# eradiate/eradiate-kernel

Measured on AMD Instinct MI355X. Metric: Msamples/s volpath 512x512x1024spp plane-parallel atmosphere, higher is better.
Workload: dtype f32; 1 GPU; C3 volpath heterogeneous 128^3 grid + HG g=0.8, 512x512x1024spp; integrator=volpath, sampler=independent seed 0, block_size=32, rfilter=box

## Files before the change

eradiate-kernel_amd/csrc/volpath_flat.h:

```cpp
#pragma once
#include "integrator_dev.h"

namespace mtsamd {
inline namespace MTS_VARIANT_NS {

#if MTS_SPEC_N == 3
#define MTS_CX
#define MTS_CXI(id)
#define MTS_SPEC_DW 3
#else
#define MTS_CX , cx
#define MTS_CXI(id) , cx, (id)
#define MTS_SPEC_DW 4
#endif

#if MTS_SPEC_N == 3
#define MTS_FILM_STRIDE(sc) ((size_t) 5)
#else
#define MTS_FILM_STRIDE(sc) ((size_t) (sc).film_channels)
#endif
#ifndef MTS_CHAIN
#define MTS_CHAIN 1
#endif
#ifndef MTS_REPEAT_MIN_W
// ... 140 lines not shown
        if (COUNT) cnt.n_lookup++;
        if (COUNT) MTS_SEG(cnt, 2);
    }
    mi.combined = combined;
    mi.inv_combined = inv_mext;
    mi.info = (m_homogeneous ? MI_HOMOGENEOUS : 0u) | (m_spectral ? MI_SPECTRAL : 0u) |
              (m.sample_emitters ? MI_SAMPLE_EMITTERS : 0u) | (m_grey ? MI_GREY : 0u) | ((uint32_t) m.phase << MI_PHASE_SHIFT);
    return mi;
}

DEV Spec transmittance_exp_g(float t, Spec combined, bool grey) {
    if (grey) return spec_s(pm_exp(-t * combined.x));
    return transmittance_exp(t, combined);
}

#if MTS_SPEC_N == 3
template <bool OWN_ATOMIC>
DEV void splat_sample_t(const DScene &sc, const DBlock &blk, uint32_t lx, uint32_t ly, F2 position_sample, F3 L, bool valid,
                        MTS_GLOBAL_AS float *film, float *own) {
    const DSensor &se = sc.sensor;
    float v[5];
    v[0] = pm_fma(0.180423f, L.z, pm_fma(0.357580f, L.y, 0.412453f * L.x));
    v[1] = pm_fma(0.072169f, L.z, pm_fma(0.715160f, L.y, 0.212671f * L.x));
    v[2] = pm_fma(0.950227f, L.z, pm_fma(0.119193f, L.y, 0.019334f * L.x));
    if (sc.integrator.monochrome)
        v[0] = v[1] = v[2] = L.x;
    v[3] = valid ? 1.f : 0.f;
    v[4] = 1.f;
    bool ok = true;
    for (int k = 0; k < 5; ++k) ok = ok && v[k] >= -1e-5f && pm_isfinite(v[k]);
    if (!ok) return;
    const DRFilter &rf = se.rfilter;
    const int border = rf.border_size;
    const int sx = blk.sx + 2 * border, sy = blk.sy + 2 * border;
    float posx = position_sample.x - ((float) (blk.ox - border) + .5f), posy = position_sample.y - ((float) (blk.oy - border) + .5f);
    if (rf.radius > 0.5f + MTS_RAY_EPSILON) {
        int lox = max((int) pm_ceil(posx - rf.radius), 0), loy = max((int) pm_ceil(posy - rf.radius), 0);
        int hix = min((int) pm_floor(posx + rf.radius), sx - 1), hiy = min((int) pm_floor(posy + rf.radius), sy - 1);
        uint32_t n = (uint32_t) pm_ceil((rf.radius - 2.f * MTS_RAY_EPSILON) * 2.f);
        float basex = (float) lox - posx, basey = (float) loy - posy;
        for (uint32_t yr = 0; yr < n; ++yr) {
            int y = loy + (int) yr;
            if (y > hiy) break;
            float wy = as_global(rf.values)[min((int) pm_abs((basey + (float) yr) * rf.scale_factor), 31)];
            int fy = blk.oy - border + y - se.crop_y;
            for (uint32_t xr = 0; xr < n; ++xr) {
                int x = lox + (int) xr;
                if (x > hix) break;
                float wx = as_global(rf.values)[min((int) pm_abs((basex + (float) xr) * rf.scale_factor), 31)];
                float weight = wy * wx;
                int fx = blk.ox - border + x - se.crop_x;
                if (fx >= 0 && fy >= 0 && fx < se.crop_w && fy < se.crop_h) {
                    float *dst = (float *) (film + 5 * ((size_t) fy * se.crop_w + fx));
                    for (int k = 0; k < 5; ++k) atomicAdd(dst + k, v[k] * weight);
                }
            }
        }
    } else {
        int lox = (int) pm_ceil(posx - .5f), loy = (int) pm_ceil(posy - .5f);
        if (lox == (int) lx && loy == (int) ly) {
            if (OWN_ATOMIC) { for (int k = 0; k < 5; ++k) atomicAdd(own + k, v[k]); }
            else { for (int k = 0; k < 5; ++k) own[k] += v[k]; }
        } else if (lox >= 0 && loy >= 0 && lox < sx && loy < sy) {
            float *dst = (float *) (film + 5 * ((size_t) (blk.oy + loy - se.crop_y) * se.crop_w + (blk.ox + lox - se.crop_x)));
            for (int k = 0; k < 5; ++k) atomicAdd(dst + k, v[k]);
        }
    }
}

#endif

struct PathState {
    Pcg32 rng;
    DRay ray;
    Hit si;
    int medium;
    Spec thr, res; float eta; uint32_t depth, channel;
    Spec trans; float wa, wb;
#if MTS_SPEC_N != 3
    Spec wl;
#endif
    uint32_t st, mode, flags;
};
enum { C_POS = 0,
       C_RAYW = 2,
       C_SO = 3, C_SD = 6,
       C_SHIT = 9,
       C_SMED = 17,
       C_CW = 18,
       C_EMIT = C_CW + MTS_SPEC_DW,
       C_ACC = C_EMIT + MTS_SPEC_DW,
       C_SAMPLE = C_ACC + 5,
       C_COUNT = C_SAMPLE + 1 };
static_assert(C_COUNT <= 32, "the cold record is one 128-byte line");
#define MTS_COLD_RECORD 32
template <class Ptr , bool AOS = false>
struct ColdStoreT {
    Ptr base; uint32_t stride;
    DEV auto &f(int k) const { return AOS ? base[k] : base[(size_t) k * stride]; }
    DEV void put3(int k, F3 v) const { f(k) = v.x; f(k + 1) = v.y; f(k + 2) = v.z; }
    DEV F3 get3(int k) const { return f3(f(k), f(k + 1), f(k + 2)); }
#if MTS_SPEC_N == 3
    DEV void put_spec(int k, Spec v) const { put3(k, v); }
    DEV Spec get_spec(int k) const { return get3(k); }
#else
    DEV void put_spec(int k, Spec v) const { f(k) = v.x; f(k + 1) = v.y; f(k + 2) = v.z; f(k + 3) = v.w; }
    DEV Spec get_spec(int k) const { return spec4(f(k), f(k + 1), f(k + 2), f(k + 3)); }
#endif
    DEV void put_hit(const Hit &h) const {
        f(C_SHIT) = h.t; put3(C_SHIT + 1, h.p); f(C_SHIT + 4) = h.uv.x; f(C_SHIT + 5) = h.uv.y;
        f(C_SHIT + 6) = __int_as_float(h.shape); f(C_SHIT + 7) = __int_as_float(h.prim);
    }
    DEV Hit get_hit() const {
        Hit h; h.t = f(C_SHIT); h.p = get3(C_SHIT + 1); h.uv.x = f(C_SHIT + 4); h.uv.y = f(C_SHIT + 5);
        h.shape = __float_as_int(f(C_SHIT + 6)); h.prim = __float_as_int(f(C_SHIT + 7)); return h;
    }
};
typedef ColdStoreT<float *> ColdStore;
typedef ColdStoreT<MTS_GLOBAL_AS float *, true> ColdStoreHbm;
template <class Cold>
struct PathEnvT {
    DBlock blk; uint32_t lx, ly, sample_count; MTS_GLOBAL_AS float *film; Cold cold;
    MTS_GLOBAL_AS float *park;
    uint32_t index;
};
enum { B_INT = 0, B_MED , B_SCATTER, B_WSURF, B_SURF, B_PHASE, B_NEW,
       B_MEDW , B_DONE, B_COUNT };

template <bool COUNT>
struct VolpathMachine {
    const DScene &sc;
    Counters &cnt;
    DEV VolpathMachine(const DScene &sc_, Counters &cnt_) : sc(sc_), cnt(cnt_) {}
#if MTS_SPEC_N == 3
    DEV SpecCtx ctx(const PathState &) const { return SpecCtx(); }
#else
    DEV SpecCtx ctx(const PathState &p) const { SpecCtx cx = make_ctx(sc); cx.wl = p.wl; return cx; }
#endif

    DEV void queue_intersection(PathState &p) const {
        float bmint, bmaxt;
        bbox_ray_intersect(sc.bbox, p.ray, bmint, bmaxt);
        p.si.t = pm_inf();
        if (pm_max(p.ray.mint, bmint) <= bmaxt) p.flags |= FL_NEEDS_INT; else p.flags &= ~FL_NEEDS_INT;
    }
    template <class E> DEV void begin_sample(PathState &p, const E &e) const {
        const DSensor &se = sc.sensor;
        const float px = (float) (e.lx + (uint32_t) e.blk.ox), py = (float) (e.ly + (uint32_t) e.blk.oy);
        if (se.wavefront) seed_wavefront_sample(p.rng, se, e.blk, e.lx, e.ly, __float_as_uint(e.cold.f(C_SAMPLE)));
        F2 u = p.rng.next_2d();
        F2 position_sample; position_sample.x = px + u.x; position_sample.y = py + u.y;
        F2 aperture_sample; aperture_sample.x = .5f; aperture_sample.y = .5f;
        if (se.needs_aperture_sample) aperture_sample = p.rng.next_2d();
        if (se.shutter_open_time > 0.f) (void) p.rng.next_1d();
#if MTS_SPEC_N == 3
        (void) p.rng.next_1d();
#else
        {
            const float wavelength_sample = p.rng.next_1d();
            float wav_weight; Spec srf_weight;
            p.wl = sc.srf >= 0 ? sample_wavelengths_srf(sc, wavelength_sample, srf_weight) : sample_wavelengths(wavelength_sample, wav_weight);
        }
#endif
        F2 adjusted;
        adjusted.x = (position_sample.x - (float) se.crop_x) / (float) se.crop_w;
        adjusted.y = (position_sample.y - (float) se.crop_y) / (float) se.crop_h;
        F3 rw;
        p.ray = sensor_sample_ray(sc, adjusted, aperture_sample, rw);
        e.cold.f(C_POS) = position_sample.x; e.cold.f(C_POS + 1) = position_sample.y; e.cold.f(C_RAYW) = rw.x;
        p.medium = se.medium;
        p.thr = spec_s(1.f); p.res = spec_s(0.f); p.eta = 1.f; p.depth = 0;
#if MTS_SPEC_N == 3
        p.channel = sc.integrator.monochrome ? 0u : (uint32_t) pm_min(p.rng.next_1d() * 3.f, 2.f);
#else
        p.channel = 0u;
#endif
        p.si.p = f3s(0.f); p.si.uv.x = p.si.uv.y = 0.f; p.si.prim = 0;
        const bool hide_emitters = sc.integrator.hide_emitters != 0;
        p.flags = FL_ALIVE | ((!hide_emitters && sc.environment >= 0) ? FL_VALID_RAY : 0u) | (!hide_emitters ? FL_SPEC_CHAIN : 0u);
        p.trans = spec_s(1.f); p.wa = p.wb = 0.f;
        queue_intersection(p);
        p.mode = M_MAIN; p.st = S_TOP;
    }
    template <class E> DEV void end_nee(PathState &p, const E &e) const {
        Spec emitted = p.trans * e.cold.get_spec(C_EMIT);
        p.res = p.res + e.cold.get_spec(C_CW) * emitted;
        p.mode = M_MAIN; p.medium = __float_as_int(e.cold.f(C_SMED));
        F3 d = e.cold.get3(C_SD);
        p.ray.d = d; p.ray.d_rcp = vrcp(d);
        if (p.flags & FL_FROM_MEDIUM) { p.ray.o = e.cold.get3(C_SO); p.st = S_PHASE; }
        else { p.si = e.cold.get_hit(); p.st = S_BSDF; }
    }
    template <class E> DEV void end_direct(PathState &p, const E &e, Spec emitter_val, float emitter_pdf) const {
        Spec emitted = p.trans * emitter_val;
        if (emitter_pdf != 0.f) p.res = p.res + mis_weight(p.wb, emitter_pdf) * p.thr * emitted;
        p.ray = spawn_ray(e.cold.get3(C_SO), e.cold.get3(C_SD));
        p.si = e.cold.get_hit(); p.medium = __float_as_int(e.cold.f(C_SMED));
        p.flags = (p.flags & ~FL_NEEDS_INT) | FL_ALIVE;
        p.mode = M_MAIN; p.st = S_TOP;
    }

    template <bool DEFER = false, class E> DEV void top(PathState &p, const E &e) const {
        if (p.st != S_TOP) return;
        const uint32_t max_depth = (uint32_t) sc.integrator.max_depth, rr_depth = (uint32_t) sc.integrator.rr_depth;
        if (p.mode == M_MAIN) {
            bool active = (p.flags & FL_ALIVE) && any_nonzero(p.thr);
            float q = pm_min(hmax(p.thr) * (p.eta * p.eta), .95f);
            bool perform_rr = p.depth > rr_depth;
            active = active && (p.rng.next_1d() < q || !perform_rr);
            if (perform_rr) p.thr = p.thr * pm_rcp(q);
            if (!active || p.depth >= max_depth) p.st = S_NEW;
            else { if (COUNT) cnt.n_iter++; p.st = p.medium >= 0 ? S_MED : S_SURF; }
        } else if (p.mode == M_NEE) {
            float remaining_dist = p.wb * (1.f - MTS_SHADOW_EPSILON) - p.wa;
            p.ray.maxt = remaining_dist;
            if (!(remaining_dist > 0.f)) { if (DEFER) p.st = S_ENDNEE; else end_nee(p, e); }
            else { if (COUNT) cnt.n_nee_step++; p.st = p.medium >= 0 ? S_MED : S_SURF; }
        } else {
            if (COUNT) cnt.n_nee_step++;
            p.st = p.medium >= 0 ? S_MED : S_SURF;
        }
    }
    DEV static bool wants_int(const PathState &p) { return (p.st == S_MED || p.st == S_SURF || p.st == S_DIRB) && (p.flags & FL_NEEDS_INT); }
    DEV static int classify(const PathState &p) {
        if (p.st == S_DONE) return B_DONE;
        if (wants_int(p)) return B_INT;
        if (p.st == S_MED) return p.mode == M_MAIN ? B_MED : B_MEDW;
        if (p.st == S_SCATTER) return B_SCATTER;
        if (p.st == S_SURF) return p.mode == M_MAIN ? B_SURF : B_WSURF;
        if (p.st == S_BSDF) return B_SURF;
        if (p.st == S_PHASE) return B_PHASE;
        return B_NEW;
    }

    template <class E> DEV void blk_new(PathState &p, const E &e) const {
        if (p.st != S_NEW) return;
        const DSensor &se = sc.sensor;
        F2 position_sample; position_sample.x = e.cold.f(C_POS); position_sample.y = e.cold.f(C_POS + 1);
        float acc[5];
        for (int k = 0; k < 5; ++k) acc[k] = e.cold.f(C_ACC + k);
#if MTS_SPEC_N == 3
        splat_sample_t<false>(sc, e.blk, e.lx, e.ly, position_sample, f3s(e.cold.f(C_RAYW)) * p.res, (p.flags & FL_VALID_RAY) != 0, e.film, acc);
#else
        {
            float wav_weight; (void) sample_wavelengths(0.f, wav_weight);
            const Spec ww = sc.srf >= 0 ? srf_weights_of(sc, p.wl) : spec_s(wav_weight);
            const Spec L = (ww * e.cold.f(C_RAYW)) * p.res;
            float xyz[3];
            spectrum_to_xyz(sc.cie, L, p.wl, xyz);
            const float v[5] = { xyz[0], xyz[1], xyz[2], (p.flags & FL_VALID_RAY) != 0 ? 1.f : 0.f, 1.f };
            if (sc.bin_count == 0) splat_values_t<false>(sc, e.blk, e.lx, e.ly, position_sample, v, e.film, acc);
            else splat_values_bins(sc, e.blk, e.lx, e.ly, position_sample, v, p.res, p.wl, e.film, acc);
        }
#endif
        const uint32_t sample_idx = __float_as_uint(e.cold.f(C_SAMPLE)) + 1u;
        if (sample_idx == e.sample_count) {
            float *own = (float *) (e.film + MTS_FILM_STRIDE(sc) * ((size_t) (e.blk.oy + (int) e.ly - se.crop_y) * se.crop_w + (e.blk.ox + (int) e.lx - se.crop_x)));
            for (int k = 0; k < 5; ++k) atomicAdd(own + k, acc[k]);
            p.st = S_DONE;
        } else {
            for (int k = 0; k < 5; ++k) e.cold.f(C_ACC + k) = acc[k];
            e.cold.f(C_SAMPLE) = __uint_as_float(sample_idx);
            begin_sample(p, e);
        }
    }
    template <class E> DEV void blk_int(PathState &p, const E &e) const {
        if (!wants_int(p)) return;
        p.si = ray_intersect(sc, p.ray);
        p.flags &= ~FL_NEEDS_INT;
        start_direct(p, e);
    }
    template <class E> DEV void start_direct(PathState &p, const E &e) const {
        if (p.st != S_DIRB || (p.flags & FL_NEEDS_INT)) return;
// ... 23 lines not shown
        const Spec sigma_n = homogeneous ? spec_s(0.f) : mi.combined - mi.sigma_t;
        const uint32_t channel = p.channel;
        const bool is_main = MODEK == 0 ? true : (MODEK == 1 ? false : p.mode == M_MAIN), is_nee = MODEK == 0 ? false : p.mode == M_NEE;
        const float remaining_dist = is_nee ? p.ray.maxt : pm_inf();
        Spec weight = is_main ? p.thr : p.trans;
        if (spectral) {
            float t = pm_min(mi.t, p.si.t);
            if (is_nee) t = pm_min(remaining_dist, t);
            t = t - mi.mint;
            const bool surface_first = p.si.t < mi.t || mi.t > remaining_dist;
            if (grey || !homogeneous) {
                float tr = pm_exp(-t * mi.combined.x);
                float tr_pdf = surface_first ? tr : tr * mi.combined.x;
                weight = weight * (tr_pdf > 0.f ? tr * pm_rcp(tr_pdf) : 0.f);
            } else {
                Spec tr = transmittance_exp(t, mi.combined);
                Spec free_flight_pdf = surface_first ? tr : tr * mi.combined;
                float tr_pdf = pick(free_flight_pdf, channel);
                weight = weight * (tr_pdf > 0.f ? tr / tr_pdf : spec_s(0.f));
            }
        }
        float u2 = 0.f;
        if (is_main) u2 = p.rng.next_1d();
        if (is_nee) {
            if (mi.t > remaining_dist && mi.t != pm_inf()) p.wa = p.wb;
            if (mi.t > remaining_dist) mi.t = pm_inf();
        }
        const bool valid = mi.t != pm_inf();
        if (!valid) {
            if (is_main) p.thr = weight; else p.trans = weight;
            p.st = S_SURF;
            return;
        }
        const bool real_scatter = is_main && !(u2 >= (grey ? div_by_invariant(mi.sigma_t.x, mi.combined.x, mi.inv_combined)
                                                                : div_by_invariant(pick(mi.sigma_t, channel), pick(mi.combined, channel), mi.inv_combined)));
        if (!real_scatter) {
            if (grey) {
                if (is_main) { if (spectral) weight = weight * ((sigma_n.x * mi.combined.x) * pm_rcp(sigma_n.x)); }
                else { if (spectral) weight = weight * sigma_n.x; else weight = weight * div_by_invariant(sigma_n.x, mi.combined.x, mi.inv_combined); }
            } else {
                if (is_main) { if (spectral) weight = weight * (sigma_n * pick(mi.combined, channel) / pick(sigma_n, channel)); }
                else { if (spectral) weight = weight * sigma_n; else weight = weight * div_by_invariant(sigma_n, mi.combined, mi.inv_combined); }
            }
            if (is_nee) p.wa += mi.t;
            p.ray.o = mi.p; p.ray.mint = 0.f; p.si.t = p.si.t - mi.t;
            p.st = S_TOP;
            if (is_main) p.thr = weight;
            else {
                p.trans = weight;
                if (!any_nonzero(weight)) {
                    if (DEFER) p.st = is_nee ? S_ENDNEE : S_ENDDIR0;
                    else if (is_nee) end_nee(p, e); else end_direct(p, e, spec_s(0.f), 0.f);
                }
            }
            return;
        }
        p.depth += 1;
        if (!(p.depth < max_depth)) { p.thr = weight; p.flags &= ~FL_ALIVE; p.st = S_TOP; return; }
        if (grey) {
            if (spectral) weight = weight * ((mi.sigma_s.x * mi.combined.x) * pm_rcp(mi.sigma_t.x));
            else weight = weight * (mi.sigma_s.x / mi.sigma_t.x);
        } else {
            if (spectral) weight = weight * (mi.sigma_s * pick(mi.combined, channel) / pick(mi.sigma_t, channel));
            else weight = weight * (mi.sigma_s / mi.sigma_t);
        }
        p.thr = weight;
        const bool sample_emitters = (mi.info & MI_SAMPLE_EMITTERS) != 0;
        p.flags |= FL_VALID_RAY;
        p.flags = sample_emitters ? (p.flags & ~FL_SPEC_CHAIN) : (p.flags | FL_SPEC_CHAIN);
        p.ray.o = mi.p;
        p.st = sample_emitters ? S_SCATTER : S_PHASE;
    }
    template <class E> DEV void blk_scatter(PathState &p, const E &e) const {
        if (p.st != S_SCATTER) return;
        p.st = S_PHASE;
        Spec emitter_val;
        const SpecCtx cx = ctx(p); (void) cx;
        DirSample ds = sample_emitter_direction(sc, p.ray.o, p.rng.next_2d(), false, emitter_val MTS_CX);
        if (ds.pdf == 0.f) return;
        float phase_val = 0.f;
        WATERFALL_BEGIN(p.medium, mu)
            phase_val = phase_eval<true>(sc, cload(sc.media + mu).phase, -p.ray.d, p.ray.o, ds.d MTS_CX);
        WATERFALL_END
        e.cold.put_spec(C_CW, p.thr * phase_val); e.cold.put_spec(C_EMIT, emitter_val);
        e.cold.put3(C_SO, p.ray.o); e.cold.put3(C_SD, p.ray.d); e.cold.f(C_SMED) = __int_as_float(p.medium);
        p.trans = spec_s(1.f); p.wa = 0.f; p.wb = ds.dist;
        p.ray = spawn_ray(p.ray.o, ds.d); p.ray.mint = 0.f;
        queue_intersection(p);
        p.flags |= FL_FROM_MEDIUM;
        p.mode = M_NEE; p.st = S_TOP;
    }
    template <class E> DEV void blk_wsurf(PathState &p, const E &e) const {
        if (p.st != S_SURF || p.mode == M_MAIN || (p.flags & FL_NEEDS_INT)) return;
        const bool hit = hit_valid(p.si);
        const bool is_nee = p.mode == M_NEE;
        if (is_nee) p.wa += p.si.t;
        int emitter = is_nee ? -1 : sc.environment;
        Surf sf; sf.wi = -p.ray.d; sf.sh.n = f3s(0.f); sf.n = f3s(0.f);
        Spec nt = spec_s(0.f); int is_tr = 0, ext = -1, inte = -1;
        if (hit) {
            WATERFALL_BEGIN(p.si.shape, su)
                const DShape s = cload(sc.shapes + su);
                if (!is_nee) emitter = s.emitter;
                nt = s.bsdf_type == MTS_BSDF_NULL ? spec_s(1.f) : spec_s(0.f);
                is_tr = s.is_medium_transition; ext = s.exterior; inte = s.interior;
                if (emitter >= 0) complete_surface(sc, s, p.si, p.ray.d, sf);
                else if (is_tr) sf.n = hit_geo_normal(sc, s, p.si);
            WATERFALL_END
        }
        if (emitter >= 0) {
            const F3 ref_p = e.cold.get3(C_SO);
            DirSample ds;
            ds.p = p.si.p; ds.n = sf.sh.n; ds.d = p.si.p - ref_p; ds.dist = norm(ds.d); ds.d = ds.d / ds.dist;
            if (!hit) ds.d = -sf.wi;
            ds.emitter = emitter; ds.pdf = 0.f; ds.delta = false;
            const SpecCtx cx = ctx(p); (void) cx;
            end_direct(p, e, emitter_eval(sc, emitter, sf.wi.z MTS_CX), pdf_emitter_direction(sc, ref_p, ds));
            return;
        }
        if (hit) {
            p.trans = p.trans * nt;
            p.ray = spawn_ray(p.si.p, p.ray.d);
            queue_intersection(p);
            if (is_tr) p.medium = dot(p.ray.d, sf.n) > 0 ? ext : inte;
        }
        if (hit && any_nonzero(p.trans)) p.st = S_TOP;
        else if (is_nee) end_nee(p, e);
        else end_direct(p, e, spec_s(0.f), 0.f);
    }
    template <class E> DEV void blk_surf(PathState &p, const E &e) const {
        if (p.st != S_SURF || p.mode != M_MAIN || (p.flags & FL_NEEDS_INT)) return;
        const uint32_t max_depth = (uint32_t) sc.integrator.max_depth;
        const bool hit = hit_valid(p.si);
        Surf sf; sf.wi = -p.ray.d; sf.n = f3s(0.f); sf.sh.s = sf.sh.t = sf.sh.n = f3s(0.f);
        int emitter = sc.environment, bsdf_id = 0;
        if (hit) {
            WATERFALL_BEGIN(p.si.shape, su)
                const DShape s = cload(sc.shapes + su);
                emitter = s.emitter; bsdf_id = s.bsdf;
                if (s.emitter >= 0 || (s.bsdf_flags & F_Smooth) != 0) complete_surface(sc, s, p.si, p.ray.d, sf);
            WATERFALL_END
        }
        const SpecCtx cx = ctx(p); (void) cx;
        if ((p.flags & FL_SPEC_CHAIN) && emitter >= 0) p.res = p.res + p.thr * emitter_eval(sc, emitter, sf.wi.z MTS_CX);
        if (!hit) { p.flags &= ~FL_ALIVE; p.st = S_TOP; return; }
        p.st = S_BSDF;
        bool active_e = false;
        WATERFALL_BEGIN(bsdf_id, bu)
            active_e = (cload(sc.bsdfs + bu).flags & F_Smooth) != 0 && (p.depth + 1 < max_depth);
        WATERFALL_END
        if (!active_e) return;
        Spec emitter_val;
        DirSample ds = sample_emitter_direction(sc, p.si.p, p.rng.next_2d(), false, emitter_val MTS_CX);
        if (ds.pdf == 0.f) return;
        F3 wo = to_local(sf.sh, ds.d);
        Spec bsdf_val; float bpdf;
        WATERFALL_BEGIN(bsdf_id, bu)
            const DBsdf bsdf = cload(sc.bsdfs + bu);
            bsdf_val = bsdf_eval(bsdf, sf.wi, wo MTS_CXI(bu));
            bpdf = bsdf_pdf(bsdf, sf.wi, wo MTS_CXI(bu));
        WATERFALL_END
        e.cold.put_spec(C_CW, p.thr * bsdf_val * mis_weight(ds.pdf, ds.delta ? 0.f : bpdf)); e.cold.put_spec(C_EMIT, emitter_val);
        e.cold.put_hit(p.si); e.cold.put3(C_SD, p.ray.d); e.cold.f(C_SMED) = __int_as_float(p.medium);
        p.trans = spec_s(1.f); p.wa = 0.f; p.wb = ds.dist;
        p.ray = spawn_ray(p.si.p, ds.d);
        queue_intersection(p);
        p.flags &= ~FL_FROM_MEDIUM;
        p.mode = M_NEE; p.st = S_TOP;
    }
    template <class E> DEV void blk_bsdf(PathState &p, const E &e) const {
        if (p.st != S_BSDF) return;
        const uint32_t max_depth = (uint32_t) sc.integrator.max_depth;
        Surf sf; int bsdf_id = 0, is_tr = 0, ext = -1, inte = -1;
        WATERFALL_BEGIN(p.si.shape, su)
            const DShape s = cload(sc.shapes + su);
            complete_surface(sc, s, p.si, p.ray.d, sf);
            bsdf_id = s.bsdf; is_tr = s.is_medium_transition; ext = s.exterior; inte = s.interior;
        WATERFALL_END
        const float s1 = p.rng.next_1d(); const F2 s2 = p.rng.next_2d();
        BSDFSample bs; Spec bsdf_val;
        const SpecCtx cx = ctx(p); (void) cx;
        WATERFALL_BEGIN(bsdf_id, bu)
            const DBsdf bsdf = cload(sc.bsdfs + bu);
            bsdf_val = bsdf_sample(bsdf, sf.wi, s1, s2, bs MTS_CXI(bu));
        WATERFALL_END
        p.thr = p.thr * bsdf_val;
        p.eta *= bs.eta;
        p.ray = spawn_ray(p.si.p, to_world(sf.sh, bs.wo));
        p.flags |= FL_ALIVE;
        const bool non_null_bsdf = !(bs.sampled_type & F_Null);
        if (non_null_bsdf) { p.depth += 1; p.flags |= FL_VALID_RAY; }
        if (non_null_bsdf && (bs.sampled_type & F_Delta)) p.flags |= FL_SPEC_CHAIN;
        if (bs.sampled_type & F_Smooth) p.flags &= ~FL_SPEC_CHAIN;
        const bool add_emitter = !(bs.sampled_type & F_Delta) && any_nonzero(p.thr) && (p.depth < max_depth);
        const int new_medium = is_tr ? (dot(p.ray.d, sf.n) > 0 ? ext : inte) : p.medium;
        queue_intersection(p);
        if (add_emitter) { e.cold.f(C_SMED) = __int_as_float(new_medium); p.wb = bs.pdf; p.st = S_DIRB; start_direct(p, e); }
        else { p.medium = new_medium; p.st = S_TOP; }
    }
    template <class E> DEV void blk_phase(PathState &p, const E &e) const {
        if (p.st != S_PHASE) return;
        const float s1 = p.rng.next_1d(); const F2 s2 = p.rng.next_2d();
        F3 wo;
        const SpecCtx cx = ctx(p); (void) cx;
        WATERFALL_BEGIN(p.medium, mu)
            wo = phase_sample<true>(sc, cload(sc.media + mu).phase, make_frame(p.ray.d), p.ray.o, s1, s2 MTS_CX);
        WATERFALL_END
        p.ray = spawn_ray(p.ray.o, wo); p.ray.mint = 0.0f;
        queue_intersection(p);
        p.flags |= FL_ALIVE;
        p.st = S_TOP;
    }

    template <class E> DEV void finish(PathState &p, const E &e) const {
        if (p.st == S_ENDNEE) end_nee(p, e);
        else if (p.st == S_ENDDIR0) end_direct(p, e, spec_s(0.f), 0.f);
    }
    template <bool DEFER = false, bool SPLIT = false, class E> DEV void run(PathState &p, const E &e, int sel) const {
        switch (sel) {
            case B_NEW: blk_new(p, e); break;
            case B_INT: blk_int(p, e); break;
            case B_MED: if (SPLIT) blk_med<DEFER, 0>(p, e); else blk_med<DEFER, -1>(p, e); break;
            case B_MEDW: if (SPLIT) blk_med<DEFER, 1>(p, e); else blk_med<DEFER, -1>(p, e); break;
            case B_SCATTER: blk_scatter(p, e); break;
            case B_WSURF: blk_wsurf(p, e); break;
            case B_SURF: blk_surf(p, e); blk_bsdf(p, e); break;
            case B_PHASE: blk_phase(p, e); break;
            default: break;
        }
    }
};

#if MTS_SPEC_N == 3
template <bool COUNT>
DEV void volpath_pixel_flat(const DScene &sc, Pcg32 &rng, const DBlock &blk, uint32_t lx, uint32_t ly, uint32_t sample_count,
                            float *__restrict__ film, ColdStore cold, Counters &cnt, const uint32_t *stop_flag) {
    VolpathMachine<COUNT> vm(sc, cnt);
    PathEnvT<ColdStore> e; e.blk = blk; e.lx = lx; e.ly = ly; e.sample_count = sample_count; e.film = as_global(film); e.cold = cold;
    PathState p; p.rng = rng;
    for (int k = 0; k < 5; ++k) e.cold.f(C_ACC + k) = 0.f;
    e.cold.f(C_SAMPLE) = __uint_as_float(0u);
    vm.begin_sample(p, e);
#if defined(MTSAMD_BLOCKSTATS)
    long long bs_t0 = clock64(); int bs_prev_sel = 20;
    unsigned long long bs_loc[45] = {};
// ... 516 lines not shown
```

eradiate-kernel_amd/csrc/volpathmis_flat.h:

```cpp
#pragma once
#include "volpath_flat.h"

namespace mtsamd {
inline namespace MTS_VARIANT_NS {

#if MTS_SPEC_N == 3
DEV int c_pdfv(bool) { return 30; }
#else
DEV int c_pdfv(bool from_medium) { return from_medium ? C_SHIT : C_SO; }
#endif

template <bool SPEC>
struct MisPathState {
    Pcg32 rng;
    DRay ray; Hit si; int medium;
    MisWeights<SPEC> pf, pn;
    MisWeights<SPEC> wn, wu;
    Spec res; F3 lsp;
#if MTS_SPEC_N != 3
    Spec wl;
#endif
    float eta, wa, wb;
    uint32_t depth, channel, st, mode, flags;
};

template <bool COUNT, bool SPEC>
struct VolpathMisMachine {
    typedef MisPathState<SPEC> P;
    typedef MisWeights<SPEC> W;
    const DScene &sc;
    Counters &cnt;
    DEV VolpathMisMachine(const DScene &sc_, Counters &cnt_) : sc(sc_), cnt(cnt_) {}
#if MTS_SPEC_N == 3
    DEV SpecCtx ctx(const P &) const { return SpecCtx(); }
#else
    DEV SpecCtx ctx(const P &p) const { SpecCtx cx = make_ctx(sc); cx.wl = p.wl; return cx; }
#endif

    DEV void queue_intersection(P &p) const {
        float bmint, bmaxt;
        bbox_ray_intersect(sc.bbox, p.ray, bmint, bmaxt);
        p.si.t = pm_inf();
        if (pm_max(p.ray.mint, bmint) <= bmaxt) p.flags |= FL_NEEDS_INT; else p.flags &= ~FL_NEEDS_INT;
    }
    template <class E> DEV static void park_put(const E &e, const W &a, const W &b) {
        constexpr int NR = SPEC ? MTS_SPEC_N : 1;
        for (int i = 0; i < NR; ++i) {
            MTS_GLOBAL_AS float *pa = e.park + MTS_SPEC_N * i, *pb = e.park + MTS_SPEC_N * (NR + i);
            pa[0] = a.r[i].x; pa[1] = a.r[i].y; pa[2] = a.r[i].z; pb[0] = b.r[i].x; pb[1] = b.r[i].y; pb[2] = b.r[i].z;
#if MTS_SPEC_N != 3
            pa[3] = a.r[i].w; pb[3] = b.r[i].w;
#endif
        }
    }
    template <class E> DEV static void park_get(const E &e, W &a, W &b) {
        constexpr int NR = SPEC ? MTS_SPEC_N : 1;
        for (int i = 0; i < NR; ++i) {
            const MTS_GLOBAL_AS float *pa = e.park + MTS_SPEC_N * i, *pb = e.park + MTS_SPEC_N * (NR + i);
            a.r[i].x = pa[0]; a.r[i].y = pa[1]; a.r[i].z = pa[2]; b.r[i].x = pb[0]; b.r[i].y = pb[1]; b.r[i].z = pb[2];
#if MTS_SPEC_N != 3
            a.r[i].w = pa[3]; b.r[i].w = pb[3];
#endif
        }
    }
    DEV bool walk_goes_on(const P &p) const {
        if (SPEC) return any_nonzero(mis_weight_w(p.wu));
        return any_nonzero(p.wu.r[0]) || any_nonzero(p.wn.r[0]);
    }
    template <class E> DEV void begin_sample(P &p, const E &e) const {
        const DSensor &se = sc.sensor;
        const float px = (float) (e.lx + (uint32_t) e.blk.ox), py = (float) (e.ly + (uint32_t) e.blk.oy);
        if (se.wavefront) seed_wavefront_sample(p.rng, se, e.blk, e.lx, e.ly, __float_as_uint(e.cold.f(C_SAMPLE)));
        F2 u = p.rng.next_2d();
        F2 position_sample; position_sample.x = px + u.x; position_sample.y = py + u.y;
        F2 aperture_sample; aperture_sample.x = .5f; aperture_sample.y = .5f;
        if (se.needs_aperture_sample) aperture_sample = p.rng.next_2d();
        if (se.shutter_open_time > 0.f) (void) p.rng.next_1d();
#if MTS_SPEC_N == 3
        (void) p.rng.next_1d();
#else
        {
            const float wavelength_sample = p.rng.next_1d();
            float wav_weight; Spec srf_weight;
            p.wl = sc.srf >= 0 ? sample_wavelengths_srf(sc, wavelength_sample, srf_weight) : sample_wavelengths(wavelength_sample, wav_weight);
        }
#endif
        F2 adjusted;
        adjusted.x = (position_sample.x - (float) se.crop_x) / (float) se.crop_w;
        adjusted.y = (position_sample.y - (float) se.crop_y) / (float) se.crop_h;
        F3 rw;
        p.ray = sensor_sample_ray(sc, adjusted, aperture_sample, rw);
        e.cold.f(C_POS) = position_sample.x; e.cold.f(C_POS + 1) = position_sample.y; e.cold.f(C_RAYW) = rw.x;
        p.medium = se.medium;
        p.res = spec_s(0.f); p.lsp = f3s(0.f); p.eta = 1.f; p.depth = 0;
        p.pf = mw_full<SPEC>(1.f); p.pn = mw_full<SPEC>(1.f); p.wn = mw_full<SPEC>(1.f); p.wu = mw_full<SPEC>(1.f);
#if MTS_SPEC_N == 3
        p.channel = sc.integrator.monochrome ? 0u : (uint32_t) pm_min(p.rng.next_1d() * 3.f, 2.f);
#else
        p.channel = 0u;
#endif
        p.si.p = f3s(0.f); p.si.uv.x = p.si.uv.y = 0.f; p.si.prim = 0; p.si.shape = -1;
        const bool hide_emitters = sc.integrator.hide_emitters != 0;
        p.flags = FL_ALIVE | ((!hide_emitters && sc.environment >= 0) ? FL_VALID_RAY : 0u) | (!hide_emitters ? FL_SPEC_CHAIN : 0u);
        p.wa = p.wb = 0.f;
        queue_intersection(p);
        p.mode = M_MAIN; p.st = S_TOP;
    }
    template <class E> DEV void end_nee(P &p, const E &e) const {
        const Spec fval = e.cold.get_spec(C_CW), emitted = e.cold.get_spec(C_EMIT);
        const float pdfv = e.cold.f(c_pdfv((p.flags & FL_FROM_MEDIUM) != 0));
        update_weights(p.wn, 1.0f, fval, p.channel, true);
        update_weights(p.wu, pdfv, fval, p.channel, true);
        p.res = p.res + mis_weight_w(p.wn, p.wu) * emitted;
        park_get(e, p.pf, p.pn);
        p.mode = M_MAIN; p.medium = __float_as_int(e.cold.f(C_SMED));
        F3 d = e.cold.get3(C_SD);
        p.ray.d = d; p.ray.d_rcp = vrcp(d);
        if (p.flags & FL_FROM_MEDIUM) { p.ray.o = e.cold.get3(C_SO); p.st = S_PHASE; }
        else { p.si = e.cold.get_hit(); p.st = S_BSDF; }
    }
    template <bool DEFER, class E> DEV void nee_done(P &p, const E &e) const { if (DEFER) p.st = S_ENDNEE; else end_nee(p, e); }
    template <class E> DEV void finish(P &p, const E &e) const { if (p.st == S_ENDNEE) end_nee(p, e); }
    template <bool DEFER = false, class E> DEV void top(P &p, const E &e) const {
        if (p.st != S_TOP) return;
        const uint32_t max_depth = (uint32_t) sc.integrator.max_depth, rr_depth = (uint32_t) sc.integrator.rr_depth;
        if (p.mode == M_MAIN) {
            bool active = (p.flags & FL_ALIVE) != 0;
            Spec mis_throughput = mis_weight_w(p.pf);
            float q = pm_min(hmax(mis_throughput) * (p.eta * p.eta), .95f);
            bool perform_rr = active && (p.depth > rr_depth);
            active = active && !(p.rng.next_1d() >= q && perform_rr);
            update_weights(p.pf, q, 1.0f, p.channel, perform_rr);
            active = active && !(p.depth >= max_depth);
            active = active && any_nonzero(mis_weight_w(p.pf));
            if (!active) p.st = S_NEW;
            else { if (COUNT) cnt.n_iter++; p.st = p.medium >= 0 ? S_MED : S_SURF; }
        } else {
            float remaining_dist = p.wb * (1.f - MTS_SHADOW_EPSILON) - p.wa;
            p.ray.maxt = remaining_dist;
            if (!(remaining_dist > 0.f)) nee_done<DEFER>(p, e);
            else { if (COUNT) cnt.n_nee_step++; p.st = p.medium >= 0 ? S_MED : S_SURF; }
        }
    }
    DEV static bool wants_int(const P &p) { return (p.st == S_MED || p.st == S_SURF) && (p.flags & FL_NEEDS_INT); }
    DEV static int classify(const P &p) {
        if (p.st == S_DONE) return B_DONE;
        if (wants_int(p)) return B_INT;
        if (p.st == S_MED) return p.mode == M_MAIN ? B_MED : B_MEDW;
        if (p.st == S_SCATTER) return B_SCATTER;
        if (p.st == S_SURF) return p.mode == M_MAIN ? B_SURF : B_WSURF;
        if (p.st == S_BSDF) return B_SURF;
        if (p.st == S_PHASE) return B_PHASE;
        return B_NEW;
    }

    template <class E> DEV void blk_new(P &p, const E &e) const {
        if (p.st != S_NEW) return;
        const DSensor &se = sc.sensor;
        F2 position_sample; position_sample.x = e.cold.f(C_POS); position_sample.y = e.cold.f(C_POS + 1);
        float acc[5];
        for (int k = 0; k < 5; ++k) acc[k] = e.cold.f(C_ACC + k);
#if MTS_SPEC_N == 3
        splat_sample_t<false>(sc, e.blk, e.lx, e.ly, position_sample, f3s(e.cold.f(C_RAYW)) * p.res, (p.flags & FL_VALID_RAY) != 0, e.film, acc);
#else
        {
            float wav_weight; (void) sample_wavelengths(0.f, wav_weight);
            const Spec ww = sc.srf >= 0 ? srf_weights_of(sc, p.wl) : spec_s(wav_weight);
            const Spec L = (ww * e.cold.f(C_RAYW)) * p.res;
            float xyz[3];
            spectrum_to_xyz(sc.cie, L, p.wl, xyz);
            const float v[5] = { xyz[0], xyz[1], xyz[2], (p.flags & FL_VALID_RAY) != 0 ? 1.f : 0.f, 1.f };
            if (sc.bin_count == 0) splat_values_t<false>(sc, e.blk, e.lx, e.ly, position_sample, v, e.film, acc);
            else splat_values_bins(sc, e.blk, e.lx, e.ly, position_sample, v, p.res, p.wl, e.film, acc);
        }
#endif
        const uint32_t sample_idx = __float_as_uint(e.cold.f(C_SAMPLE)) + 1u;
        if (sample_idx == e.sample_count) {
            float *own = (float *) (e.film + MTS_FILM_STRIDE(sc) * ((size_t) (e.blk.oy + (int) e.ly - se.crop_y) * se.crop_w + (e.blk.ox + (int) e.lx - se.crop_x)));
            for (int k = 0; k < 5; ++k) atomicAdd(own + k, acc[k]);
            p.st = S_DONE;
        } else {
            for (int k = 0; k < 5; ++k) e.cold.f(C_ACC + k) = acc[k];
            e.cold.f(C_SAMPLE) = __uint_as_float(sample_idx);
            begin_sample(p, e);
        }
    }
    template <class E> DEV void blk_int(P &p, const E &) const {
        if (!wants_int(p)) return;
        p.si = ray_intersect(sc, p.ray);
        p.flags &= ~FL_NEEDS_INT;
    }
    template <class E> DEV void blk_med(P &p, const E &) const {
        if (p.st != S_MED || p.mode != M_MAIN || (p.flags & FL_NEEDS_INT)) return;
        const uint32_t max_depth = (uint32_t) sc.integrator.max_depth, channel = p.channel;
        const float u = p.rng.next_1d();
        MedStep mi;
        const SpecCtx cx = ctx(p); (void) cx;
        WATERFALL_BEGIN(p.medium, mu)
            mi = medium_step<COUNT>(sc, cload(sc.media + mu), p.ray, u, channel, true, cnt MTS_CX);
        WATERFALL_END
        if (p.si.t < mi.t) mi.t = pm_inf();
#if MTS_TRAITS & MT_MEDIA
        const bool spectral = true, homogeneous = false, grey = MTS_SPEC_N == 3;
#elif MTS_TRAITS & MT_HOMOG
        const bool spectral = (mi.info & MI_SPECTRAL) != 0, homogeneous = true, grey = (mi.info & MI_GREY) != 0;
#else
        const bool spectral = (mi.info & MI_SPECTRAL) != 0, homogeneous = (mi.info & MI_HOMOGENEOUS) != 0, grey = (mi.info & MI_GREY) != 0;
#endif
        const Spec sigma_n = homogeneous ? spec_s(0.f) : mi.combined - mi.sigma_t;
        if (spectral) {
            float t = pm_min(mi.t, p.si.t) - mi.mint;
            if (homogeneous) {
                Spec tr = transmittance_exp(t, mi.combined);
                Spec free_flight_pdf = p.si.t < mi.t ? tr : tr * mi.combined;
                update_weights(p.pf, free_flight_pdf, tr, channel, true);
                update_weights(p.pn, free_flight_pdf, tr, channel, true);
            } else {
                const float tr = pm_exp(-t * mi.combined.x), free_flight_pdf = p.si.t < mi.t ? tr : tr * mi.combined.x;
                update_weights_uniform(p.pf, free_flight_pdf, tr);
                update_weights_uniform(p.pn, free_flight_pdf, tr);
            }
        }
        if (mi.t == pm_inf()) { p.st = S_SURF; return; }
        const bool null_scatter = p.rng.next_1d() >= div_by_invariant(pick(mi.sigma_t, channel), pick(mi.combined, channel), mi.inv_combined);
        if (null_scatter) {
            if (spectral && grey) {
                update_weights_uniform(p.pf, div_by_invariant(sigma_n.x, mi.combined.x, mi.inv_combined), sigma_n.x);
                update_weights_uniform(p.pn, 1.0f, sigma_n.x);
            } else if (spectral) {
                update_weights(p.pf, div_by_invariant(sigma_n, mi.combined, mi.inv_combined), sigma_n, channel, true);
                update_weights(p.pn, 1.0f, sigma_n, channel, true);
            } else {
                update_weights(p.pf, sigma_n, sigma_n, channel, true);
                update_weights(p.pn, 1.0f, div_by_invariant(sigma_n, mi.combined, mi.inv_combined), channel, true);
            }
            p.ray.o = mi.p; p.ray.mint = 0.f; p.si.t = p.si.t - mi.t;
            p.st = S_TOP;
            return;
        }
        p.depth += 1; p.lsp = mi.p;
        const bool sample_emitters = (mi.info & MI_SAMPLE_EMITTERS) != 0;
        if (!(p.depth < max_depth)) { p.flags &= ~FL_ALIVE; p.st = S_TOP; return; }
        if (sample_emitters) p.flags &= ~FL_SPEC_CHAIN;
        if (spectral && grey) update_weights_uniform(p.pf, div_by_invariant(mi.sigma_t.x, mi.combined.x, mi.inv_combined), mi.sigma_s.x);
        else if (spectral) update_weights(p.pf, div_by_invariant(mi.sigma_t, mi.combined, mi.inv_combined), mi.sigma_s, channel, true);
        else update_weights(p.pf, mi.sigma_t, mi.sigma_s, channel, true);
        p.flags |= FL_VALID_RAY;
        p.ray.o = mi.p;
        p.st = sample_emitters ? S_SCATTER : S_PHASE;
    }
    template <bool DEFER, class E> DEV void start_walk(P &p, const E &e, F3 ref_p, const DirSample &ds, Spec emitter_sample_weight, Spec fval, float pdfv, bool from_medium) const {
        park_put(e, p.pf, p.pn);
        p.wn = p.pf; p.wu = p.pf;
        Spec emitter_val = emitter_sample_weight * ds.pdf;
        if (ds.pdf == 0.f) emitter_val = spec_s(0.f);
        const bool active = ds.pdf != 0.f;
        update_weights(p.wn, ds.pdf, 1.0f, p.channel, active);
        e.cold.put_spec(C_CW, fval); e.cold.put_spec(C_EMIT, emitter_val);
        e.cold.put3(C_SD, p.ray.d); e.cold.f(C_SMED) = __int_as_float(p.medium);
        if (from_medium) { e.cold.put3(C_SO, p.ray.o); p.flags |= FL_FROM_MEDIUM; }
        else { e.cold.put_hit(p.si); p.flags &= ~FL_FROM_MEDIUM; }
        e.cold.f(c_pdfv(from_medium)) = pdfv;
        p.mode = M_NEE;
        if (!active) { nee_done<DEFER>(p, e); return; }
        p.wa = 0.f; p.wb = ds.dist;
        p.ray = spawn_ray(ref_p, ds.d);
        if (from_medium) p.ray.mint = 0.f;
        queue_intersection(p);
        p.st = S_TOP;
    }
    template <bool DEFER = false, class E> DEV void blk_scatter(P &p, const E &e) const {
        if (p.st != S_SCATTER) return;
        Spec esw;
        const SpecCtx cx = ctx(p); (void) cx;
        DirSample ds = sample_emitter_direction(sc, p.ray.o, p.rng.next_2d(), false, esw MTS_CX);
        float phase_val = 0.f;
        WATERFALL_BEGIN(p.medium, mu)
            phase_val = phase_eval<true>(sc, cload(sc.media + mu).phase, -p.ray.d, p.ray.o, ds.d MTS_CX);
        WATERFALL_END
        start_walk<DEFER>(p, e, p.ray.o, ds, esw, spec_s(phase_val), ds.delta ? 0.f : phase_val, true);
    }
    template <bool DEFER = false, class E> DEV void blk_medw(P &p, const E &e) const {
        if (p.st != S_MED || p.mode == M_MAIN || (p.flags & FL_NEEDS_INT)) return;
        const uint32_t channel = p.channel;
        const float u = p.rng.next_1d();
        MedStep mi;
        const SpecCtx cx = ctx(p); (void) cx;
        WATERFALL_BEGIN(p.medium, mu)
            mi = medium_step<COUNT>(sc, cload(sc.media + mu), p.ray, u, channel, false, cnt MTS_CX);
        WATERFALL_END
        if (p.si.t < mi.t) mi.t = pm_inf();
#if MTS_TRAITS & MT_MEDIA
        const bool spectral = true, homogeneous = false, grey = MTS_SPEC_N == 3;
#elif MTS_TRAITS & MT_HOMOG
        const bool spectral = (mi.info & MI_SPECTRAL) != 0, homogeneous = true, grey = (mi.info & MI_GREY) != 0;
#else
        const bool spectral = (mi.info & MI_SPECTRAL) != 0, homogeneous = (mi.info & MI_HOMOGENEOUS) != 0, grey = (mi.info & MI_GREY) != 0;
#endif
        const Spec sigma_n = homogeneous ? spec_s(0.f) : mi.combined - mi.sigma_t;
        const float remaining_dist = p.ray.maxt;
        if (spectral) {
            float t = pm_min(remaining_dist, pm_min(mi.t, p.si.t)) - mi.mint;
            const bool no_event = p.si.t < mi.t || mi.t > remaining_dist;
            if (homogeneous) {
                Spec tr = transmittance_exp(t, mi.combined);
                Spec free_flight_pdf = no_event ? tr : tr * mi.combined;
                update_weights(p.wn, free_flight_pdf, tr, channel, true);
                update_weights(p.wu, free_flight_pdf, tr, channel, true);
            } else {
                const float tr = pm_exp(-t * mi.combined.x), free_flight_pdf = no_event ? tr : tr * mi.combined.x;
                update_weights_uniform(p.wn, free_flight_pdf, tr);
                update_weights_uniform(p.wu, free_flight_pdf, tr);
            }
        }
        if (mi.t > remaining_dist && mi.t != pm_inf()) p.wa = p.wb;
        if (mi.t > remaining_dist) mi.t = pm_inf();
        if (mi.t == pm_inf()) { p.st = S_SURF; return; }
        p.wa += mi.t;
        p.ray.o = mi.p; p.ray.mint = 0.f; p.si.t = p.si.t - mi.t;
        if (spectral && grey) {
            update_weights_uniform(p.wn, 1.f, sigma_n.x);
            update_weights_uniform(p.wu, div_by_invariant(sigma_n.x, mi.combined.x, mi.inv_combined), sigma_n.x);
        } else if (spectral) {
            update_weights(p.wn, 1.f, sigma_n, channel, true);
            update_weights(p.wu, div_by_invariant(sigma_n, mi.combined, mi.inv_combined), sigma_n, channel, true);
        } else {
            update_weights(p.wn, 1.f, div_by_invariant(sigma_n, mi.combined, mi.inv_combined), channel, true);
            update_weights(p.wu, sigma_n, sigma_n, channel, true);
        }
        if (walk_goes_on(p)) p.st = S_TOP; else nee_done<DEFER>(p, e);
    }
    template <class E> DEV void blk_wsurf(P &p, const E &e) const {
        if (p.st != S_SURF || p.mode == M_MAIN || (p.flags & FL_NEEDS_INT)) return;
        const bool hit = hit_valid(p.si);
        p.wa += p.si.t;
        if (!hit) { end_nee(p, e); return; }
        Spec nt = spec_s(0.f); F3 n = f3s(0.f); int is_tr = 0, ext = -1, inte = -1;
        WATERFALL_BEGIN(p.si.shape, su)
            const DShape s = cload(sc.shapes + su);
            nt = s.bsdf_type == MTS_BSDF_NULL ? spec_s(1.f) : spec_s(0.f);
            is_tr = s.is_medium_transition; ext = s.exterior; inte = s.interior;
// ... 390 lines not shown
```

Before: 638.2 Msamples/s.

## Repack cold path record so each NEE flavour uses aligned 16-byte groups in one half

```diff
diff --git a/eradiate-kernel_amd/csrc/volpath_flat.h b/eradiate-kernel_amd/csrc/volpath_flat.h
--- a/eradiate-kernel_amd/csrc/volpath_flat.h
+++ b/eradiate-kernel_amd/csrc/volpath_flat.h
@@ -246,17 +246,31 @@
 #endif
     uint32_t st, mode, flags;
 };
-enum { C_POS = 0,
-       C_RAYW = 2,
-       C_SO = 3, C_SD = 6,
-       C_SHIT = 9,
-       C_SMED = 17,
-       C_CW = 18,
-       C_EMIT = C_CW + MTS_SPEC_DW,
-       C_ACC = C_EMIT + MTS_SPEC_DW,
-       C_SAMPLE = C_ACC + 5,
-       C_COUNT = C_SAMPLE + 1 };
+enum { C_SD = 0,
+       C_SMED = 3,
+       C_SO = 4,
+       C_PV = 7,
+       C_EMIT = 8,
+       C_CWM = 12,
+       C_SHIT = 8,
+       C_CWS = 4,
+       C_WALK_END = 16,
+       C_EMITS = 16,
+       C_POS = 20,
+       C_RAYW = 22,
+       C_SAMPLE = 23,
+       C_ACC = 24,
+       C_PDFVS = 29,
+       C_COUNT = 30 };
 static_assert(C_COUNT <= 32, "the cold record is one 128-byte line");
+static_assert(C_SMED == C_SD + 3 && C_PV == C_SO + 3 && C_SAMPLE == C_RAYW + 1 && C_RAYW == C_POS + 2, "fields that share one wide access are neighbours");
+static_assert(C_SD % 4 == 0 && C_SO % 4 == 0 && C_EMIT % 4 == 0 && C_CWM % 4 == 0 && C_SHIT % 4 == 0 && C_CWS % 4 == 0 && C_EMITS % 4 == 0 &&
+              C_POS % 4 == 0 && C_ACC % 4 == 0, "every group of the cold record starts on a 16-byte boundary");
+static_assert(C_PV + 1 <= C_EMIT && C_EMIT + MTS_SPEC_DW <= C_CWM && C_CWM + MTS_SPEC_DW <= C_WALK_END, "medium-started NEE: inside the walk half");
+static_assert(C_PV + 1 <= C_SHIT && C_SHIT + 8 <= C_WALK_END, "direct-light walk: inside the walk half");
+static_assert(C_SMED + 1 <= C_CWS && C_CWS + MTS_SPEC_DW <= C_SHIT, "surface-started NEE: the weight fits between the head and the hit");
+static_assert(C_EMITS >= C_WALK_END && C_EMITS + MTS_SPEC_DW <= C_POS && C_POS >= C_WALK_END && C_ACC + 5 <= C_PDFVS && C_PDFVS < C_COUNT,
+              "the sample half: overflow of the surface-started NEE, then the sample's own fields");
 #define MTS_COLD_RECORD 32
 template <class Ptr , bool AOS = false>
 struct ColdStoreT {
@@ -347,12 +361,16 @@
         p.mode = M_MAIN; p.st = S_TOP;
     }
     template <class E> DEV void end_nee(PathState &p, const E &e) const {
-        Spec emitted = p.trans * e.cold.get_spec(C_EMIT);
-        p.res = p.res + e.cold.get_spec(C_CW) * emitted;
+        const bool from_medium = (p.flags & FL_FROM_MEDIUM) != 0;
+        static_assert(C_CWS == C_SO && C_PV == C_SO + 3, "end_nee reads C_SO / C_PV and C_CWS as one group");
+        const Spec w47 = e.cold.get_spec(C_CWS); const float pv = e.cold.f(C_PV);
+        const Spec emitted = p.trans * e.cold.get_spec(from_medium ? C_EMIT : C_EMITS);
+        const Spec weight = from_medium ? p.thr * pv : w47;
+        p.res = p.res + weight * emitted;
         p.mode = M_MAIN; p.medium = __float_as_int(e.cold.f(C_SMED));
         F3 d = e.cold.get3(C_SD);
         p.ray.d = d; p.ray.d_rcp = vrcp(d);
-        if (p.flags & FL_FROM_MEDIUM) { p.ray.o = e.cold.get3(C_SO); p.st = S_PHASE; }
+        if (from_medium) { p.ray.o = f3(w47.x, w47.y, w47.z); p.st = S_PHASE; }
         else { p.si = e.cold.get_hit(); p.st = S_BSDF; }
     }
     template <class E> DEV void end_direct(PathState &p, const E &e, Spec emitter_val, float emitter_pdf) const {
@@ -542,8 +560,9 @@
         WATERFALL_BEGIN(p.medium, mu)
             phase_val = phase_eval<true>(sc, cload(sc.media + mu).phase, -p.ray.d, p.ray.o, ds.d MTS_CX);
         WATERFALL_END
-        e.cold.put_spec(C_CW, p.thr * phase_val); e.cold.put_spec(C_EMIT, emitter_val);
-        e.cold.put3(C_SO, p.ray.o); e.cold.put3(C_SD, p.ray.d); e.cold.f(C_SMED) = __int_as_float(p.medium);
+        e.cold.put3(C_SD, p.ray.d); e.cold.f(C_SMED) = __int_as_float(p.medium);
+        e.cold.put3(C_SO, p.ray.o); e.cold.f(C_PV) = phase_val;
+        e.cold.put_spec(C_EMIT, emitter_val);
         p.trans = spec_s(1.f); p.wa = 0.f; p.wb = ds.dist;
         p.ray = spawn_ray(p.ray.o, ds.d); p.ray.mint = 0.f;
         queue_intersection(p);
@@ -620,7 +639,7 @@
             bsdf_val = bsdf_eval(bsdf, sf.wi, wo MTS_CXI(bu));
             bpdf = bsdf_pdf(bsdf, sf.wi, wo MTS_CXI(bu));
         WATERFALL_END
-        e.cold.put_spec(C_CW, p.thr * bsdf_val * mis_weight(ds.pdf, ds.delta ? 0.f : bpdf)); e.cold.put_spec(C_EMIT, emitter_val);
+        e.cold.put_spec(C_CWS, p.thr * bsdf_val * mis_weight(ds.pdf, ds.delta ? 0.f : bpdf)); e.cold.put_spec(C_EMITS, emitter_val);
         e.cold.put_hit(p.si); e.cold.put3(C_SD, p.ray.d); e.cold.f(C_SMED) = __int_as_float(p.medium);
         p.trans = spec_s(1.f); p.wa = 0.f; p.wb = ds.dist;
         p.ray = spawn_ray(p.si.p, ds.d);
diff --git a/eradiate-kernel_amd/csrc/volpathmis_flat.h b/eradiate-kernel_amd/csrc/volpathmis_flat.h
--- a/eradiate-kernel_amd/csrc/volpathmis_flat.h
+++ b/eradiate-kernel_amd/csrc/volpathmis_flat.h
@@ -4,11 +4,9 @@
 namespace mtsamd {
 inline namespace MTS_VARIANT_NS {
 
-#if MTS_SPEC_N == 3
-DEV int c_pdfv(bool) { return 30; }
-#else
-DEV int c_pdfv(bool from_medium) { return from_medium ? C_SHIT : C_SO; }
-#endif
+DEV int c_pdfv(bool from_medium) { return from_medium ? C_PV : C_PDFVS; }
+DEV int c_cw(bool from_medium) { return from_medium ? C_CWM : C_CWS; }
+DEV int c_emit(bool from_medium) { return from_medium ? C_EMIT : C_EMITS; }
 
 template <bool SPEC>
 struct MisPathState {
@@ -107,8 +105,9 @@
         p.mode = M_MAIN; p.st = S_TOP;
     }
     template <class E> DEV void end_nee(P &p, const E &e) const {
-        const Spec fval = e.cold.get_spec(C_CW), emitted = e.cold.get_spec(C_EMIT);
-        const float pdfv = e.cold.f(c_pdfv((p.flags & FL_FROM_MEDIUM) != 0));
+        Spec fval, emitted; float pdfv;
+        if (p.flags & FL_FROM_MEDIUM) { fval = e.cold.get_spec(C_CWM); emitted = e.cold.get_spec(C_EMIT); pdfv = e.cold.f(C_PV); }
+        else { fval = e.cold.get_spec(C_CWS); emitted = e.cold.get_spec(C_EMITS); pdfv = e.cold.f(C_PDFVS); }
         update_weights(p.wn, 1.0f, fval, p.channel, true);
         update_weights(p.wu, pdfv, fval, p.channel, true);
         p.res = p.res + mis_weight_w(p.wn, p.wu) * emitted;
@@ -256,7 +255,7 @@
         if (ds.pdf == 0.f) emitter_val = spec_s(0.f);
         const bool active = ds.pdf != 0.f;
         update_weights(p.wn, ds.pdf, 1.0f, p.channel, active);
-        e.cold.put_spec(C_CW, fval); e.cold.put_spec(C_EMIT, emitter_val);
+        e.cold.put_spec(c_cw(from_medium), fval); e.cold.put_spec(c_emit(from_medium), emitter_val);
         e.cold.put3(C_SD, p.ray.d); e.cold.f(C_SMED) = __int_as_float(p.medium);
         if (from_medium) { e.cold.put3(C_SO, p.ray.o); p.flags |= FL_FROM_MEDIUM; }
         else { e.cold.put_hit(p.si); p.flags &= ~FL_FROM_MEDIUM; }
```

Result: no change. 636.3 Msamples/s (-0.3%).
